# Lumina-Group/libzkp

Hardware: AMD Instinct MI355X
Metric: proofs/sec (whole node) + ms/proof p50, 4096-proof mixed batch (range / equality / membership / improvement) per MI355X (higher is better)
Workload: dtype u32/u64 integer limbs (10x25.5-bit GF(2^255-19), BN254 Fq on 9x29-bit limbs in the MSM loops and 10x26-bit elsewhere, 8x32-bit Fr and scalars mod l, 2x64-bit f128)

## Files before the change

### libzkp_amd/csrc/g16_impl.inc

```

namespace {

struct G16Key {
    bool loaded = false;
    uint32_t n_inst = 0, n_wit = 0, nv = 0, n_rows = 0, m = 0, logm = 0;
    G16Circuit C{};
    std::vector<void*> allocs;
    uint32_t *table_g1 = nullptr, *table_g2 = nullptr;
    G16Radix rx = g16_radix(G16_WBITS_DEFAULT);
    int shared_tables = -1;
    uint64_t table_bytes = 0;
    struct Chunking { DevLayout lay; const uint32_t* corr = nullptr; const uint16_t* scal = nullptr; };
    std::vector<SlotList> targets_g1, targets_g2;
    std::vector<uint16_t> hscal_g1, hscal_g2;
    std::map<uint64_t, Chunking> lays_g1, lays_g2;
    uint64_t win_g1 = 0, win_g2 = 0;
    const uint32_t *init_g1 = nullptr, *init_g2 = nullptr;
    G16Vk vk{}; bool vk_ready = false;
    uint64_t vk_table_bytes = 0;
    bool verifier_only() const { return vk_ready && !loaded; }
    const uint32_t *vm_kconst = nullptr, *vm_lines = nullptr;
};
struct G16Run {
    void* buf = nullptr; size_t cap = 0; hipStream_t side = nullptr, side2 = nullptr; hipEvent_t ev[4] = {nullptr, nullptr, nullptr, nullptr};
// ... 316 lines not shown
    const HostR1CS cs = kind == G16_EQUALITY ? build_equality_r1cs() : build_membership_r1cs();
    const HostCircuitTables T = build_circuit_tables(cs);
    uint32_t seed[8];
    if (setup_seed) memcpy(seed, setup_seed, 32);
    else { std::vector<uint8_t> f; int rc0 = fresh_seeds(f, 1); if (rc0) return rc0; memcpy(seed, f.data(), 32); }
    const char* tagname = kind == G16_EQUALITY ? "equality_mimc" : "membership_mimc";
    uint8_t th[32]; sha256_host(th, (const uint8_t*)tagname, strlen(tagname));
    const uint32_t tag = (uint32_t)th[0] | ((uint32_t)th[1] << 8) | ((uint32_t)th[2] << 16);
    fr tw[5];
    for (uint32_t k = 0; k < 5; k++) { tw[k] = tape_fr(seed, 0x47313601u, 8 * tag + k); if (fp_is_zero(tw[k])) tw[k] = fp_one<FrParams>(); }
    const fr alpha = tw[0], beta = tw[1], gamma = tw[2], delta = tw[3], tau = tw[4];
    const uint32_t m = T.m, nv = T.nv;
    const fr one = fp_one<FrParams>();
    fr taum = one; for (uint32_t i = 0; i < m; i++) taum = fp_mul(taum, tau);
    const fr zt = fp_sub(taum, one), minv = fp_inv(fp_from_u64<FrParams>(m));
    const fr w = fr9_to_fr<FrParams>(ld_fr9_c(T.tw.data(), 1));
    std::vector<fr> lag(m);
    fr wj = one;
    for (uint32_t j = 0; j < m; j++) { lag[j] = fp_mul(fp_mul(fp_mul(zt, minv), wj), fp_inv(fp_sub(tau, wj))); wj = fp_mul(wj, w); }
    std::vector<fr> At(nv, fp_zero<FrParams>()), Bt = At, Ct = At;
    std::vector<fr>* dst[3] = {&At, &Bt, &Ct};
    for (int q = 0; q < 3; q++)
        for (uint32_t j = 0; j < T.n_rows; j++)
            for (uint32_t e = T.ptr[q][j]; e < T.ptr[q][j + 1]; e++)
                (*dst[q])[T.col[q][e]] = fp_add((*dst[q])[T.col[q][e]], fp_mul(ld_fr_c(T.coef[q].data(), e), lag[j]));
    for (uint32_t i = 0; i < T.n_inst; i++) At[i] = fp_add(At[i], lag[T.n_rows + i]);
    const fr ginv = fp_inv(gamma), dinv = fp_inv(delta);
    auto mix = [&](uint32_t k) { return fp_add(fp_add(fp_mul(beta, At[k]), fp_mul(alpha, Bt[k])), Ct[k]); };
    std::vector<fr> s1 = {alpha, beta, delta}, s2 = {beta, gamma, delta};
    for (uint32_t i = 0; i < T.n_inst; i++) s1.push_back(fp_mul(mix(i), ginv));
    for (uint32_t k = 0; k < nv; k++) s1.push_back(At[k]);
    for (uint32_t k = 0; k < nv; k++) s1.push_back(Bt[k]);
    { fr tp = fp_mul(zt, dinv); for (uint32_t i = 0; i + 1 < m; i++) { s1.push_back(tp); tp = fp_mul(tp, tau); } }
    for (uint32_t k = T.n_inst; k < nv; k++) s1.push_back(fp_mul(mix(k), dinv));
    for (uint32_t k = 0; k < nv; k++) s2.push_back(Bt[k]);
    std::vector<uint8_t> b1, b2; int rc;
    if ((rc = gpu_scalar_mults(false, s1, b1)) || (rc = gpu_scalar_mults(true, s2, b2))) return rc;
    auto g1at = [&](size_t i) { return b1.data() + 64 * i; };
    auto g2at = [&](size_t i) { return b2.data() + 128 * i; };
    auto put = [](std::vector<uint8_t>& v, const uint8_t* p, size_t n) { v.insert(v.end(), p, p + n); };
    auto put_len = [](std::vector<uint8_t>& v, uint64_t n) { for (int i = 0; i < 8; i++) v.push_back((uint8_t)(n >> (8 * i))); };
    size_t o_abc = 3, o_a = o_abc + T.n_inst, o_b = o_a + nv, o_h = o_b + nv, o_l = o_h + (m - 1);
    vk.clear();
    put(vk, g1at(0), 64); put(vk, g2at(0), 128); put(vk, g2at(1), 128); put(vk, g2at(2), 128);
    put_len(vk, T.n_inst); put(vk, g1at(o_abc), 64ull * T.n_inst);
    pk = vk;
    put(pk, g1at(1), 64); put(pk, g1at(2), 64);
    put_len(pk, nv); put(pk, g1at(o_a), 64ull * nv);
    put_len(pk, nv); put(pk, g1at(o_b), 64ull * nv);
    put_len(pk, nv); put(pk, g2at(3), 128ull * nv);
    put_len(pk, m - 1); put(pk, g1at(o_h), 64ull * (m - 1));
    put_len(pk, T.n_wit); put(pk, g1at(o_l), 64ull * T.n_wit);
    return load_key_locked(kind, pk.data(), pk.size());
}

int launch_msm_key(bool g2, const G16Radix& rx, const G16Key::Chunking& ch, const uint32_t* table, const uint32_t* acc_init, uint32_t rows, const uint32_t* digits, uint32_t* partial, hipStream_t st) {
    const DevLayout& D = ch.lay;
    const MsmView m = g16_msm_view(rx, D, ch.scal, table, acc_init, rows, digits, partial);
    Device::KProf& K = dev().prof[g2 ? 2 : 1];
    hipEvent_t e1 = nullptr;
    int rc = prof_begin(K, st, &e1);
    if (rc) return rc;
    ZKP_TRACED(g2 ? "k_msm_gather<G2Msm>" : "k_msm_gather<G1Msm>", st, g16_launch_msm(g2, m, st));
    prof_end(K, st, e1, D.adds_per_row * rows);
    return 0;
}


int run_g16(int kind, uint32_t rows, const uint64_t* d_value, const uint64_t* d_set_vals, const uint32_t* d_set_len, const uint8_t* d_seeds,
            uint8_t* d_out, uint64_t stride, hipStream_t st, uint32_t lane = 0) {
    G16Key& K = g16s().key[kind];
    if (!K.loaded) return no_proving_key(K);
    const uint32_t nsc = g16_nscalars(K.nv, K.m);
    const G16Key::Chunking *c1 = nullptr, *c1c = nullptr, *c2 = nullptr;
    int rc;
    if ((rc = get_chunking(K, false, G16_PART_AB, rows, &c1)) || (rc = get_chunking(K, true, G16_PART_ALL, rows, &c2))) return rc;
    if ((rc = get_chunking(K, false, G16_PART_C, rows, &c1c))) return rc;
    size_t off = 0;
    auto sz = [&](size_t bytes) { size_t o = off; off += align_up(bytes); return o; };
    const size_t W = (size_t)32 * rows;
    const size_t o_z = sz(W * K.nv), o_sd = sz((size_t)K.rx.digw * 4 * rows * nsc), o_rs = sz(W * 2), o_p1 = sz((size_t)c1->lay.nchunks * G1_JAC_W * 4 * rows),
                 o_p1c = sz((size_t)c1c->lay.nchunks * G1_JAC_W * 4 * rows), o_p2 = sz((size_t)c2->lay.nchunks * G2_JAC_W * 4 * rows),
                 o_s1 = sz((size_t)3 * G1_JAC_W * 4 * rows), o_s2 = sz((size_t)G2_JAC_W * 4 * rows), o_t1 = sz((size_t)G16_CPARTS * G1_JAC_W * 4 * rows),
                 o_qe = sz((size_t)2 * 9 * K.m * 4 * rows);
    G16Run& RW = g16s().run[kind][lane & 1u];
    if (off > RW.cap) {
        if (RW.buf) { HIP_TRY(hipDeviceSynchronize()); HIP_TRY(hipFree(RW.buf)); RW.buf = nullptr; RW.cap = 0; }
        HIP_TRY(hipMalloc(&RW.buf, off)); RW.cap = off;
    }
    uint8_t* base = (uint8_t*)RW.buf;
    G16View V{}; V.rx = K.rx; V.rows = rows; V.kind = (uint32_t)kind; V.n_inst = K.n_inst; V.n_wit = K.n_wit; V.nv = K.nv; V.m = K.m;
    V.value = d_value; V.set_vals = d_set_vals; V.set_len = d_set_len; V.seeds = reinterpret_cast<const uint32_t*>(d_seeds); V.mimc_c = g16s().mimc_dev;
    V.z = (uint32_t*)(base + o_z); V.sdig = (uint32_t*)(base + o_sd); V.rs = (uint32_t*)(base + o_rs); V.out = d_out; V.stride = stride;
    V.qap_evals = (uint32_t*)(base + o_qe);
    uint32_t *p1 = (uint32_t*)(base + o_p1), *p1c = (uint32_t*)(base + o_p1c), *p2 = (uint32_t*)(base + o_p2), *s1 = (uint32_t*)(base + o_s1), *s2 = (uint32_t*)(base + o_s2), *t1 = (uint32_t*)(base + o_t1);
    if (!RW.last) {
        for (auto& e : RW.ev) HIP_TRY(hipEventCreateWithFlags(&e, hipEventDisableTiming));
        HIP_TRY(hipEventCreateWithFlags(&RW.last, hipEventDisableTiming));
    }
    G16Run& R0 = g16s().run[kind][0];
    if (!R0.side) {
        static const int side_level = env_int("ZKP_HIP_G16_SIDE_PRIORITY", 2), side2_level = env_int("ZKP_HIP_G16_SIDE2_PRIORITY", 0);
        HIP_TRY(hipStreamCreateWithPriority(&R0.side, hipStreamNonBlocking, stream_priority(side_level)));
        HIP_TRY(hipStreamCreateWithPriority(&R0.side2, hipStreamNonBlocking, stream_priority(side2_level)));
    }
    hipStream_t const side = R0.side, side2 = R0.side2;
    hipEvent_t ev_wit = RW.ev[0], ev_ab = RW.ev[1], ev_c = RW.ev[2], ev_cp = RW.ev[3];
    ReduceView R2{}; R2.rows = rows; R2.ntargets = 1; R2.partial = p2; R2.target_chunk_begin = c2->lay.target_chunk_begin; R2.corr = c2->corr;
    if (RW.used) HIP_TRY(hipStreamWaitEvent(st, RW.last, 0));
    ZKP_TRACED("k_g16_witness", st, g16_launch_witness(V, st));
    ZKP_TRACED("k_g16_zdigits", st, g16_launch_zdigits(V, st));
    HIP_TRY(hipEventRecord(ev_wit, st));
    HIP_TRY(hipStreamWaitEvent(side, ev_wit, 0));
    { TraceMark tm_("k_g16_qap", side); HIP_TRY(g16_launch_qap(V, K.C, side)); }
    if ((rc = launch_msm_key(false, K.rx, *c1c, K.table_g1, K.init_g1, rows, V.sdig, p1c, side))) return rc;
    ReduceView Rc{}; Rc.rows = rows; Rc.ntargets = 1; Rc.partial = p1c; Rc.target_chunk_begin = c1c->lay.target_chunk_begin; Rc.corr = c1c->corr;
    ZKP_TRACED("k_sum_t<G1Msm>", side, g16_launch_sum(false, Rc, s1 + (size_t)2 * G1_JAC_W * rows, side));
    HIP_TRY(hipEventRecord(ev_c, side));
    if ((rc = launch_msm_key(false, K.rx, *c1, K.table_g1, K.init_g1, rows, V.sdig, p1, st))) return rc;
    ReduceView Rab{}; Rab.rows = rows; Rab.ntargets = 2; Rab.partial = p1; Rab.target_chunk_begin = c1->lay.target_chunk_begin; Rab.corr = c1->corr;
    if (c1->lay.ntargets == 3) Rab.target_chunk_end = c1->lay.target_chunk_begin + 2;
    HIP_TRY(hipEventRecord(ev_ab, st));
    HIP_TRY(hipStreamWaitEvent(side2, ev_ab, 0));
    ZKP_TRACED("k_sum_t<G1Msm>", side2, g16_launch_sum(false, Rab, s1, side2));
    ZKP_TRACED("k_g16_cparts", side2, g16_launch_cparts(V, s1, t1, side2));
    HIP_TRY(hipEventRecord(ev_cp, side2));
    if ((rc = launch_msm_key(true, K.rx, *c2, K.table_g2, K.init_g2, rows, V.sdig, p2, st))) return rc;
    ZKP_TRACED("k_sum_t<G2Msm>", st, g16_launch_sum(true, R2, s2, st));
    HIP_TRY(hipStreamWaitEvent(st, ev_c, 0));
    HIP_TRY(hipStreamWaitEvent(st, ev_cp, 0));
    ZKP_TRACED("k_g16_final", st, g16_launch_final(V, s1, s2, t1, st));
    HIP_TRY(hipGetLastError());
    HIP_TRY(hipEventRecord(RW.last, st)); RW.used = true;
    return 0;
}

int prove_g16_host(int kind, uint64_t n, const uint64_t* values, const uint64_t* sets_flat, const uint32_t* set_counts, const std::vector<uint8_t>& valid,
                   const uint8_t* seeds, uint8_t* out, uint64_t stride, uint32_t* out_len, int32_t* status) {
    if (g16s().key[kind].verifier_only()) return no_proving_key(g16s().key[kind]);
    std::vector<uint64_t> v, sv; std::vector<uint32_t> sl, idx; std::vector<uint8_t> sd;
    size_t pos = 0; int any = 0;
    memset(out, 0, stride * n);
    for (uint64_t i = 0; i < n; i++) {
        const uint32_t cnt = set_counts ? set_counts[i] : 0;
        if (valid[i]) {
            idx.push_back((uint32_t)i); v.push_back(values[i]);
            sd.insert(sd.end(), seeds + 32 * i, seeds + 32 * i + 32);
            if (kind == G16_MEMBERSHIP) { sl.push_back(cnt); for (uint32_t k = 0; k < G16_MAX_SET; k++) sv.push_back(k < cnt ? sets_flat[pos + k] : 0); }
            const uint32_t plen = kind == G16_EQUALITY ? EQUALITY_ENVELOPE_BYTES : (uint32_t)membership_envelope_bytes(cnt);
            if (plen > stride) return fail(ZKP_HIP_E_ARGUMENT, "stride too small for the proof envelope");
            out_len[i] = plen; status[i] = ZKP_HIP_OK;
        } else { out_len[i] = 0; status[i] = ZKP_HIP_INVALID_INPUT; any = 1; }
        pos += cnt;
    }
    const uint32_t rows = (uint32_t)idx.size();
    if (rows == 0) return any;
    hipStream_t st = dev().stream;
    uint64_t *d_v = nullptr, *d_sv = nullptr; uint32_t* d_sl = nullptr; uint8_t *d_sd = nullptr, *d_out = nullptr;
    DevScope mem;
    HIP_TRY(mem.alloc(&d_v, 8ull * rows)); HIP_TRY(mem.alloc(&d_sd, 32ull * rows)); HIP_TRY(mem.alloc(&d_out, stride * rows));
    HIP_TRY(hipMemcpyAsync(d_v, v.data(), 8ull * rows, hipMemcpyHostToDevice, st));
    HIP_TRY(hipMemcpyAsync(d_sd, sd.data(), 32ull * rows, hipMemcpyHostToDevice, st));
    HIP_TRY(hipMemsetAsync(d_out, 0, stride * rows, st));
    if (kind == G16_MEMBERSHIP) {
        HIP_TRY(mem.alloc(&d_sv, 8ull * sv.size())); HIP_TRY(mem.alloc(&d_sl, 4ull * rows));
        HIP_TRY(hipMemcpyAsync(d_sv, sv.data(), 8ull * sv.size(), hipMemcpyHostToDevice, st));
        HIP_TRY(hipMemcpyAsync(d_sl, sl.data(), 4ull * rows, hipMemcpyHostToDevice, st));
// ... 284 lines not shown
```

### libzkp_amd/csrc/g16_kernels.hip

```cpp
#include "g16_launch.h"
#include "msm_kernel.h"

struct G1Msm {
    static constexpr uint32_t ACC_W = G1_JAC_W, DIG_PER_WORD = 2;
    static __device__ __forceinline__ int32_t digit(uint32_t word, uint32_t w) { return (int32_t)(int16_t)(word >> (16 * (w & 1u))); }
    using Acc = g1_jac;
    static __device__ __forceinline__ Acc identity() { return jac_infinity<fq>(); }
    static constexpr uint32_t GATHER_WAVES = 3; static constexpr int GATHER_PREFETCH = 2;
    static constexpr uint32_t GATHER_W = 16, GATHER_STRIDE = 16, GATHER_PRIO = 0;
    using GAcc = g1_xyzz9;
    static __device__ __forceinline__ GAcc to_gather(const g1_jac& a) { return xyzz9_from_jac(a); }
    static __device__ __forceinline__ g1_jac from_gather(const GAcc& a) { return jac_from_xyzz9(a); }
    static __device__ __forceinline__ GAcc accumulate_entry(const GAcc& acc, int32_t d, const uint32_t* e) {
        g1_aff9 q{fq9_unpack8(e), fq9_unpack8(e + 8)};
        q.y = fq9_select(d < 0, fq9_neg_k<4>(q.y), q.y);
        return g1_mmadd9(acc, q);
    }
    static __device__ __forceinline__ void store(uint32_t* p, uint32_t idx, uint32_t row, uint32_t rows, const Acc& a) { st_g1_jac(p, idx, row, rows, a); }
    static __device__ __forceinline__ Acc load(const uint32_t* p, uint32_t idx, uint32_t row, uint32_t rows) { return ld_g1_jac(p, idx, row, rows); }
    static __device__ __forceinline__ Acc add(const Acc& a, const Acc& b) { return jac_add(a, b); }
};
struct G2Msm {
    static constexpr uint32_t ACC_W = G2_JAC_W, DIG_PER_WORD = 2;
    static __device__ __forceinline__ int32_t digit(uint32_t word, uint32_t w) { return (int32_t)(int16_t)(word >> (16 * (w & 1u))); }
    using Acc = g2_jac;
    static __device__ __forceinline__ Acc identity() { return jac_infinity<fq2>(); }
    static constexpr uint32_t GATHER_WAVES = 2; static constexpr int GATHER_PREFETCH = -1;
    static constexpr uint32_t GATHER_W = 32, GATHER_STRIDE = 32, GATHER_PRIO = 0;
    using GAcc = g2_xyzz9;
    static __device__ __forceinline__ GAcc to_gather(const g2_jac& a) { return g2_xyzz9_from_jac(a); }
    static __device__ __forceinline__ g2_jac from_gather(const GAcc& a) { return jac_from_g2_xyzz9(a); }
    static __device__ __forceinline__ GAcc accumulate_entry(const GAcc& acc, int32_t d, const uint32_t* e) {
        const g2_aff9 q{fq2_9{fq9_unpack8(e), fq9_unpack8(e + 8)}, fq2_9{fq9_unpack8(e + 16), fq9_unpack8(e + 24)}};
        return g2_mmadd9(acc, q, d < 0);
    }
    static __device__ __forceinline__ void store(uint32_t* p, uint32_t idx, uint32_t row, uint32_t rows, const Acc& a) { st_g2_jac(p, idx, row, rows, a); }
    static __device__ __forceinline__ Acc load(const uint32_t* p, uint32_t idx, uint32_t row, uint32_t rows) { return ld_g2_jac(p, idx, row, rows); }
    static __device__ __forceinline__ Acc add(const Acc& a, const Acc& b) { return jac_add(a, b); }
};


__global__ void __launch_bounds__(TW) k_g16_witness(G16View V) {
    ZKP_RAISE_PRIO();
    const uint32_t row = blockIdx.x * TW + threadIdx.x;
    if (row < V.rows) step_g16_witness(V, row);
}
__global__ void __launch_bounds__(TB) k_g16_zdigits(G16View V) {
    ZKP_RAISE_PRIO();
    const uint32_t row = blockIdx.x * TB + threadIdx.x;
    if (row < V.rows) step_g16_zdigits(V, blockIdx.y, row);
}
struct DevSync { __device__ __forceinline__ void operator()() const { __syncthreads(); } };
static constexpr int QAP_TB_MAX = 256;
__global__ void __launch_bounds__(QAP_TB_MAX) k_g16_qap(G16View V, G16Circuit C) {
    extern __shared__ uint32_t g16_lds[];
    G16Lds L; L.base = g16_lds; L.m = C.m;
    g16_qap_proof(V, C, L, V.qap_evals + (size_t)blockIdx.x * 2 * 9 * C.m, blockIdx.x, threadIdx.x, blockDim.x, DevSync());
}
__global__ void __launch_bounds__(TW) k_g16_cparts(G16View V, const uint32_t* sum_g1, uint32_t* tmp_g1) {
    ZKP_RAISE_PRIO();
    const uint32_t row = blockIdx.x * TW + threadIdx.x;
    if (row < V.rows) step_g16_cparts(V, sum_g1, tmp_g1, blockIdx.y, row);
}
__global__ void __launch_bounds__(TW) k_g16_final(G16View V, const uint32_t* sum_g1, const uint32_t* sum_g2, const uint32_t* tmp_g1) {
    ZKP_RAISE_PRIO();
    const uint32_t row = blockIdx.x * TW + threadIdx.x;
    if (row < V.rows) step_g16_final(V, sum_g1, sum_g2, tmp_g1, blockIdx.y, row);
}
__global__ void __launch_bounds__(TW) k_mimc_commit(const uint64_t* values, uint32_t n, const uint32_t* mimc_c, uint8_t* out) {
    const uint32_t i = blockIdx.x * TW + threadIdx.x;
    if (i >= n) return;
    G16View V{}; V.mimc_c = mimc_c; V.z = nullptr;
    const fr h = g16_mimc_chain(V, 0, fp_from_u64<FrParams>(values[i]), 0);
    uint32_t w[8]; fp_to_raw(w, h);
    g16_put_bytes(out + 32ull * i, w, 8);
}
constexpr uint32_t G16_TABLE_SEG = 512;
template <class F, uint32_t AFF_W>
__global__ void __launch_bounds__(TW, 2) k_g16_build_table(const uint32_t* bases, uint32_t nslots, uint32_t* table, uint32_t fmt9, G16Radix rx) {
    const uint32_t seg_len = rx.nent < G16_TABLE_SEG ? rx.nent : G16_TABLE_SEG, nseg = rx.nent / seg_len, slot_seg = rx.slot_ent / seg_len;
    const uint32_t t = blockIdx.x * TW + threadIdx.x;
    if (t >= nslots * slot_seg) return;
    const uint32_t slot = t / slot_seg, sg = t % slot_seg;
    uint32_t win = sg / nseg, seg = sg % nseg;
    if (rx.uneven && sg >= 16u * nseg) { win = sg < 18u * nseg ? 16u : 17u; seg = sg - (win == 16u ? 16u : 18u) * nseg; }
    constexpr uint32_t FW = AFF_W / 2, BATCH = 8;
    Aff<F> base;
    {
        const uint32_t* b = bases + (size_t)slot * AFF_W;
        uint32_t* bx = reinterpret_cast<uint32_t*>(&base.x); uint32_t* by = reinterpret_cast<uint32_t*>(&base.y);
        for (uint32_t k = 0; k < FW; k++) { bx[k] = b[k]; by[k] = b[FW + k]; }
    }
    Jac<F> q = jac_from_aff(base);
    for (uint32_t i = 0; i < g16_win_bit(rx, win); i++) q = jac_dbl(q);
    Jac<F> acc = q;
    {
        const uint32_t first = seg * seg_len + 1;
        int top = 31; while (top > 0 && !((first >> top) & 1u)) top--;
        for (int b = top - 1; b >= 0; b--) { acc = jac_dbl(acc); if ((first >> b) & 1u) acc = jac_add(acc, q); }
    }
    constexpr uint32_t NC = AFF_W / 10;
    const uint32_t OW = fmt9 ? 8 * NC : AFF_W;
    uint32_t* dst = table + ((size_t)slot * rx.slot_ent + g16_win_off(rx, win) + (size_t)seg * seg_len) * OW;
    for (uint32_t e0 = 0; e0 < seg_len; e0 += BATCH) {
        Jac<F> pts[BATCH]; F zp[BATCH];
        for (uint32_t k = 0; k < BATCH; k++) {
            pts[k] = acc; acc = jac_add(acc, q);
            zp[k] = k ? f_mul(zp[k - 1], pts[k].Z) : pts[k].Z;
        }
        F inv = f_inv(zp[BATCH - 1]);
        for (int k = BATCH - 1; k >= 0; k--) {
            const F zi = k ? f_mul(inv, zp[k - 1]) : inv;
            if (k) inv = f_mul(inv, pts[k].Z);
            const F zi2 = f_sq(zi);
            Aff<F> a; a.x = f_mul(pts[k].X, zi2); a.y = f_mul(pts[k].Y, f_mul(zi2, zi));
            const uint32_t* ax = reinterpret_cast<const uint32_t*>(&a.x); const uint32_t* ay = reinterpret_cast<const uint32_t*>(&a.y);
            uint32_t* o = dst + (size_t)(e0 + k) * OW;
            if (fmt9) {
                const fq* c = reinterpret_cast<const fq*>(&a);
                for (uint32_t t2 = 0; t2 < NC; t2++) fq9_pack8(o + 8 * t2, fq9_from_fq(c[t2]));
                continue;
            }
            for (uint32_t j = 0; j < FW; j++) { o[j] = ax[j]; o[FW + j] = ay[j]; }
        }
    }
}



__global__ void __launch_bounds__(TW) k_g16_serialize(bool g2, const uint32_t* jac, uint32_t rows, uint8_t* out) {
    const uint32_t row = blockIdx.x * TW + threadIdx.x;
    if (row >= rows) return;
    if (!g2) { uint32_t w[16]; g1_serialize(w, ld_g1_jac(jac, 0, row, rows)); g16_put_bytes(out + 64ull * row, w, 16); }
    else { uint32_t w[32]; g2_serialize(w, ld_g2_jac(jac, 0, row, rows)); g16_put_bytes(out + 128ull * row, w, 32); }
}

template __global__ void k_msm_gather<G1Msm>(MsmView, uint32_t, uint32_t);
template __global__ void k_msm_gather<G2Msm>(MsmView, uint32_t, uint32_t);
static constexpr uint32_t G16_SUM_ROWS = 8, G16_SUM_TB = 256;
template __global__ void k_sum_t<G1Msm, G16_SUM_ROWS, G16_SUM_TB>(ReduceView, uint32_t*);
template __global__ void k_sum_t<G2Msm, G16_SUM_ROWS, G16_SUM_TB>(ReduceView, uint32_t*);
template __global__ void k_g16_build_table<fq, 20>(const uint32_t*, uint32_t, uint32_t*, uint32_t, G16Radix);
template __global__ void k_g16_build_table<fq2, 40>(const uint32_t*, uint32_t, uint32_t*, uint32_t, G16Radix);

void g16_launch_witness(const G16View& V, hipStream_t st) { k_g16_witness<<<(V.rows + TW - 1) / TW, TW, 0, st>>>(V); }
void g16_launch_zdigits(const G16View& V, hipStream_t st) { k_g16_zdigits<<<dim3((V.rows + TB - 1) / TB, V.nv), TB, 0, st>>>(V); }
hipError_t g16_launch_qap(const G16View& V, const G16Circuit& C, hipStream_t st) {
    const size_t lds = (size_t)9 * C.m * 4;
    const uint32_t tb = C.m / 4;
    if (tb < 64 || tb > (uint32_t)QAP_TB_MAX || (tb & 63u)) return hipErrorInvalidValue;
    k_g16_qap<<<V.rows, tb, lds, st>>>(V, C);
    return hipSuccess;
}
void g16_launch_cparts(const G16View& V, const uint32_t* sum_g1, uint32_t* tmp_g1, hipStream_t st) {
    k_g16_cparts<<<dim3((V.rows + TW - 1) / TW, G16_CPARTS), TW, 0, st>>>(V, sum_g1, tmp_g1);
}
void g16_launch_final(const G16View& V, const uint32_t* sum_g1, const uint32_t* sum_g2, const uint32_t* tmp_g1, hipStream_t st) {
    k_g16_final<<<dim3((V.rows + TW - 1) / TW, 3), TW, 0, st>>>(V, sum_g1, sum_g2, tmp_g1);
}
void g16_launch_mimc(const uint64_t* values, uint32_t n, const uint32_t* mimc_c, uint8_t* out, hipStream_t st) { k_mimc_commit<<<(n + TW - 1) / TW, TW, 0, st>>>(values, n, mimc_c, out); }
void g16_launch_build_table(bool g2, const uint32_t* bases, uint32_t nslots, uint32_t* table, hipStream_t st, bool msm_form, const G16Radix& rx) {
    const uint32_t seg_len = rx.nent < G16_TABLE_SEG ? rx.nent : G16_TABLE_SEG;
    const uint32_t threads = nslots * (rx.slot_ent / seg_len);
    if (!g2) k_g16_build_table<fq, 20><<<(threads + TW - 1) / TW, TW, 0, st>>>(bases, nslots, table, msm_form ? 1u : 0u, rx);
    else k_g16_build_table<fq2, 40><<<(threads + TW - 1) / TW, TW, 0, st>>>(bases, nslots, table, msm_form ? 1u : 0u, rx);
}
uint32_t g16_table_entry_words(bool g2, bool msm_form) { return msm_form ? (g2 ? G2Msm::GATHER_W : G1Msm::GATHER_W) : (g2 ? 40u : 20u); }
uint32_t g16_msm_rows_per_block(bool) { return 256u; }
uint32_t g16_msm_blocks_per_cu(bool g2) { return g2 ? G2Msm::GATHER_WAVES : G1Msm::GATHER_WAVES; }
void g16_launch_msm(bool g2, const MsmView& m, hipStream_t st) {
    const uint32_t ngroups = (m.rows + 255u) / 256u, nblocks = m.nchunks * ngroups, grid = ((nblocks + 7) / 8) * 8;
    if constexpr (gather_lds_bytes<G2Msm>() > 0 || gather_lds_bytes<G1Msm>() > 0) {
        if (gather_lds_bytes<G1Msm>()) (void)hipFuncSetAttribute(reinterpret_cast<const void*>(k_msm_gather<G1Msm>), hipFuncAttributeMaxDynamicSharedMemorySize, (int)gather_lds_bytes<G1Msm>());
        if (gather_lds_bytes<G2Msm>()) (void)hipFuncSetAttribute(reinterpret_cast<const void*>(k_msm_gather<G2Msm>), hipFuncAttributeMaxDynamicSharedMemorySize, (int)gather_lds_bytes<G2Msm>());
    }
    if (!g2) k_msm_gather<G1Msm><<<grid, 256, gather_lds_bytes<G1Msm>(), st>>>(m, ngroups, nblocks);
    else k_msm_gather<G2Msm><<<grid, 256, gather_lds_bytes<G2Msm>(), st>>>(m, ngroups, nblocks);
}
void g16_launch_sum(bool g2, const ReduceView& R, uint32_t* sums, hipStream_t st) {
    const dim3 grid((R.rows + G16_SUM_ROWS - 1) / G16_SUM_ROWS, R.ntargets);
    if (!g2) k_sum_t<G1Msm, G16_SUM_ROWS, G16_SUM_TB><<<grid, G16_SUM_TB, 0, st>>>(R, sums);
    else k_sum_t<G2Msm, G16_SUM_ROWS, G16_SUM_TB><<<grid, G16_SUM_TB, 0, st>>>(R, sums);
}
void g16_launch_serialize(bool g2, const uint32_t* jac, uint32_t rows, uint8_t* out, hipStream_t st) { k_g16_serialize<<<(rows + TW - 1) / TW, TW, 0, st>>>(g2, jac, rows, out); }
```

### libzkp_amd/csrc/g16_steps.h

```cpp
#pragma once
#include "bn254_g.h"
#include "bn254_fr9.h"
#include "keccak.h"
#include "sc25519.h"

namespace zkp {

struct G16Radix { uint32_t wbits, nwin, nent, digw, nwin_u64, uneven, slot_ent; };
constexpr uint32_t G16_UNEVEN_TOP_ENT = 25088;
ZKP_HD inline G16Radix g16_radix(uint32_t wbits, bool uneven = false) {
    G16Radix r; r.wbits = wbits; r.nwin = (254 + wbits) / wbits; r.nent = 1u << (wbits - 1); r.nwin_u64 = (64 + wbits) / wbits; r.uneven = 0;
    r.slot_ent = r.nwin * r.nent;
    if (uneven && wbits == 14) { r.uneven = 1; r.nwin = 18; r.slot_ent = 18u * r.nent + G16_UNEVEN_TOP_ENT; }
    r.digw = (r.nwin + 1) / 2;
    return r;
}
ZKP_HD inline uint32_t g16_win_bit(const G16Radix& rx, uint32_t w) { return rx.uneven && w == 17 ? 239u : rx.wbits * w; }
ZKP_HD inline uint32_t g16_win_off(const G16Radix& rx, uint32_t w) { return (w + (rx.uneven && w == 17 ? 1u : 0u)) * rx.nent; }
ZKP_HD inline uint32_t g16_win_ent(const G16Radix& rx, uint32_t w) { return !rx.uneven || w < 16 ? rx.nent : w == 16 ? 2u * rx.nent : G16_UNEVEN_TOP_ENT; }
constexpr uint32_t G16_WBITS_DEFAULT = 14, G16_WBITS_KNEE = 13, G16_WBITS_MIN = 8, G16_WBITS_MAX = 15, G16_DIGW_MAX = 16;
static_assert(G16_WBITS_DEFAULT >= G16_WBITS_MIN && G16_WBITS_DEFAULT <= G16_WBITS_MAX, "key-table radix out of range");
ZKP_HD inline void g16_recode_uneven(uint32_t* packed, const sc& raw) {
    uint32_t carry = 0;
    ZKP_UNROLL for (int j = 0; j < 18; j++) {
        const int bit = j == 17 ? 239 : 14 * j, wb = j < 16 ? 14 : 15, wd = bit >> 5, sh = bit & 31;
        uint32_t x = wd < 8 ? raw.v[wd] >> sh : 0u;
        if (sh + wb > 32 && wd + 1 < 8) x |= raw.v[wd + 1] << (32 - sh);
        uint32_t d = (x & ((1u << wb) - 1u)) + carry;
        carry = j < 17 && d > (1u << (wb - 1)) ? 1u : 0u;
        d = (d - (carry << wb)) & 0xffffu;
        if ((j & 1) == 0) packed[j >> 1] = d; else packed[j >> 1] |= d << 16;
    }
}
ZKP_HD inline void g16_recode(uint32_t* packed, const sc& raw, const G16Radix& rx) {
    if (rx.uneven) { g16_recode_uneven(packed, raw); return; }
    switch (rx.wbits) {
        case 8: sc_recode_signed<8, 32>(packed, raw); break;
        case 9: sc_recode_signed<9, 29>(packed, raw); break;
        case 10: sc_recode_signed<10, 26>(packed, raw); break;
        case 11: sc_recode_signed<11, 24>(packed, raw); break;
        case 12: sc_recode_signed<12, 22>(packed, raw); break;
        case 13: sc_recode_signed<13, 20>(packed, raw); break;
        case 14: sc_recode_signed<14, 19>(packed, raw); break;
        default: sc_recode_signed<15, 17>(packed, raw); break;
    }
}
constexpr uint32_t G16V_WBITS = 10, G16V_NWIN = 26, G16V_NENT = 512, G16V_NWIN_U64 = 7;

constexpr uint32_t MIMC_ROUNDS = 110, G16_MAX_SET = 64;
constexpr uint32_t G16_TAPE_IDX = 0x47313600u;
enum { G16_EQUALITY = 0, G16_MEMBERSHIP = 1 };

ZKP_HD inline fr ld_fr(const uint32_t* p, uint32_t idx, uint32_t row, uint32_t rows) {
    fr r; const uint32_t* q = p + (size_t)idx * 8 * rows + row;
    ZKP_UNROLL for (int k = 0; k < 8; k++) r.v[k] = q[(size_t)k * rows];
    return r;
}
ZKP_HD inline void st_fr(uint32_t* p, uint32_t idx, uint32_t row, uint32_t rows, const fr& s) {
    uint32_t* q = p + (size_t)idx * 8 * rows + row;
    ZKP_UNROLL for (int k = 0; k < 8; k++) q[(size_t)k * rows] = s.v[k];
}
ZKP_HD inline fr ld_fr_c(const uint32_t* p, uint32_t idx) { fr r; ZKP_UNROLL for (int k = 0; k < 8; k++) r.v[k] = p[(size_t)idx * 8 + k]; return r; }
ZKP_HD inline void g16_put_bytes(uint8_t* dst, const uint32_t* w, int nwords) {
    for (int i = 0; i < nwords; i++) { dst[4 * i] = (uint8_t)w[i]; dst[4 * i + 1] = (uint8_t)(w[i] >> 8); dst[4 * i + 2] = (uint8_t)(w[i] >> 16); dst[4 * i + 3] = (uint8_t)(w[i] >> 24); }
}
ZKP_HD inline void st_fr_digits(uint32_t* d, uint32_t idx, uint32_t row, uint32_t rows, const fr& x, const G16Radix& rx) {
    sc raw; fp_to_raw(raw.v, x);
    uint32_t pk[G16_DIGW_MAX]; g16_recode(pk, raw, rx);
    uint32_t* q = d + (size_t)idx * rx.digw * rows + row;
    ZKP_UNROLL for (uint32_t k = 0; k < G16_DIGW_MAX; k++) if (k < rx.digw) q[(size_t)k * rows] = pk[k];
}

struct G16View {
    uint32_t rows, kind;
    G16Radix rx;
    uint32_t n_inst, n_wit, nv, m;
    const uint64_t* value;
    const uint64_t* set_vals;
    const uint32_t* set_len;
    const uint32_t* seeds;
    const uint32_t* mimc_c;
    uint32_t* z;
    uint32_t* sdig;
    uint32_t* rs;
    uint32_t* qap_evals;
    uint8_t* out; uint64_t stride;
};
ZKP_HD inline uint32_t g16_sc_h(const G16View& V) { return V.nv; }
ZKP_HD inline uint32_t g16_sc_r(const G16View& V) { return V.nv + V.m - 1; }
ZKP_HD inline uint32_t g16_sc_s(const G16View& V) { return V.nv + V.m; }
ZKP_HD inline uint32_t g16_sc_nrs(const G16View& V) { return V.nv + V.m + 1; }
ZKP_HD inline uint32_t g16_sc_one(const G16View& V) { return V.nv + V.m + 2; }
ZKP_HD inline uint32_t g16_nscalars(uint32_t nv, uint32_t m) { return nv + m + 3; }

ZKP_HD inline fr g16_mimc_chain(const G16View& V, uint32_t row, fr x, uint32_t wit0) {
    for (uint32_t i = 0; i < MIMC_ROUNDS; i++) {
        const fr t = fp_add(x, ld_fr_c(V.mimc_c, i));
        const fr t2 = fp_sq(t), t4 = fp_sq(t2);
        x = fp_mul(t4, t);
        if (V.z) { st_fr(V.z, wit0 + 3 * i, row, V.rows, t2); st_fr(V.z, wit0 + 3 * i + 1, row, V.rows, t4); st_fr(V.z, wit0 + 3 * i + 2, row, V.rows, x); }
    }
    return x;
}

ZKP_HD inline void step_g16_witness(const G16View& V, uint32_t row) {
    const uint32_t rows = V.rows;
    const uint64_t val = V.value[row];
    const fr one = fp_one<FrParams>(), zero = fp_zero<FrParams>();
    const fr v = fp_from_u64<FrParams>(val);
    uint8_t* o = V.out + (uint64_t)row * V.stride;
    st_fr(V.z, 0, row, rows, one);
    fr h;
    uint32_t proof_len = 256;
    if (V.kind == G16_EQUALITY) {
        st_fr(V.z, 2, row, rows, v); st_fr(V.z, 3, row, rows, v);
        h = g16_mimc_chain(V, row, v, 4);
        st_fr(V.z, 1, row, rows, h);
        o[0] = 2; o[1] = 2;
    } else {
        const uint32_t len = V.set_len[row];
        const uint64_t* sv = V.set_vals + (size_t)row * G16_MAX_SET;
        const uint32_t w0 = V.n_inst;
        st_fr(V.z, w0, row, rows, v);
        h = g16_mimc_chain(V, row, v, w0 + 1);
        st_fr(V.z, 1, row, rows, h);
        uint32_t pos = 0xffffffffu;
        for (uint32_t i = 0; i < len; i++) if (pos == 0xffffffffu && sv[i] == val) pos = i;
        const uint32_t sel0 = w0 + 1 + 3 * MIMC_ROUNDS;
        for (uint32_t i = 0; i < G16_MAX_SET; i++) {
            const bool real = i < len;
            const fr si = fp_from_u64<FrParams>(real ? sv[i] : 0);
            st_fr(V.z, 2 + i, row, rows, si);
            st_fr(V.z, 2 + G16_MAX_SET + i, row, rows, real ? one : zero);
            const bool sel = i == pos;
            st_fr(V.z, sel0 + i, row, rows, sel ? one : zero);
            st_fr(V.z, sel0 + G16_MAX_SET + i, row, rows, (sel && !real) ? one : zero);
            st_fr(V.z, sel0 + 2 * G16_MAX_SET + i, row, rows, sel ? fp_sub(v, si) : zero);
        }
        o[0] = 2; o[1] = 4;
        proof_len = 4 + 8 * len + 256;
        uint8_t* pl = o + 10;
        pl[0] = (uint8_t)len; pl[1] = (uint8_t)(len >> 8); pl[2] = (uint8_t)(len >> 16); pl[3] = (uint8_t)(len >> 24);
        for (uint32_t i = 0; i < len; i++) for (int k = 0; k < 8; k++) pl[4 + 8 * i + k] = (uint8_t)(sv[i] >> (8 * k));
    }
    for (int k = 0; k < 4; k++) { o[2 + k] = (uint8_t)(proof_len >> (8 * k)); o[6 + k] = (uint8_t)(32u >> (8 * k)); }
    uint32_t hraw[8]; fp_to_raw(hraw, h);
    g16_put_bytes(o + 10 + proof_len, hraw, 8);
    uint32_t seed[8]; ZKP_UNROLL for (int k = 0; k < 8; k++) seed[k] = V.seeds[(size_t)row * 8 + k];
    uint32_t w[16];
    tape_draw64(w, seed, G16_TAPE_IDX, 0); const fr r = fp_from_wide<FrParams>(w);
    tape_draw64(w, seed, G16_TAPE_IDX, 1); const fr s = fp_from_wide<FrParams>(w);
    st_fr_digits(V.sdig, g16_sc_r(V), row, rows, r, V.rx);
    st_fr_digits(V.sdig, g16_sc_s(V), row, rows, s, V.rx);
    st_fr_digits(V.sdig, g16_sc_nrs(V), row, rows, fp_neg(fp_mul(r, s)), V.rx);
    uint32_t* q = V.sdig + (size_t)g16_sc_one(V) * V.rx.digw * rows + row;
// ... 39 lines not shown
        else if (is_one) acc = fp_add(acc, ld_fr(z, c, row, rows));
        else acc = fp_add(acc, fp_mul(cf, ld_fr(z, c, row, rows)));
    }
    return acc;
}
ZKP_HD inline void g16_qap_load(const G16View& V, const G16Circuit& C, const G16Lds& L, uint32_t poly, uint32_t row, uint32_t tid, uint32_t nthreads) {
    const uint32_t nc = C.n_rows;
    const uint32_t *ptr = poly == 0 ? C.a_ptr : poly == 1 ? C.b_ptr : C.c_ptr, *col = poly == 0 ? C.a_col : poly == 1 ? C.b_col : C.c_col,
                   *coef = poly == 0 ? C.a_coef : poly == 1 ? C.b_coef : C.c_coef;
    for (uint32_t j = tid; j < C.m; j += nthreads) {
        fr a = fp_zero<FrParams>();
        if (j < nc) a = g16_row_dot_fast(ptr, col, coef, j, V.z, row, V.rows);
        else if (poly == 0 && j < nc + V.n_inst) a = ld_fr(V.z, j - nc, row, V.rows);
        L.st(j, fr9_from_fr(a));
    }
}
ZKP_HD inline void g16_bf_dif(fr9& u, fr9& v, const fr9& w) { const fr9 s = fr9_reduce_weak(fr9_add(u, v)); v = fr9_mul(fr9_sub_k<4>(u, v), w); u = s; }
ZKP_HD inline void g16_bf_dit(fr9& u, fr9& v, const fr9& w) { const fr9 t = fr9_mul(v, w); v = fr9_sub_k<2>(u, t); u = fr9_add(u, t); }
template <bool DIF>
ZKP_HD inline void g16_stage_single(const G16Circuit& C, const G16Lds& L, const uint32_t* tw, uint32_t half, uint32_t tid, uint32_t nthreads) {
    const uint32_t len = 2 * half, tstride = C.m / len;
    for (uint32_t k = tid; k < C.m / 2; k += nthreads) {
        const uint32_t grp = k / half, j = k % half, i0 = grp * len + j, i1 = i0 + half;
        const fr9 w = ld_fr9_c(tw, j * tstride);
        fr9 u = L.ld(i0), v = L.ld(i1);
        if (DIF) g16_bf_dif(u, v, w); else g16_bf_dit(u, v, w);
        L.st(i0, u); L.st(i1, v);
    }
}
template <bool DIF>
ZKP_HD inline void g16_stage_pair(const G16Circuit& C, const G16Lds& L, const uint32_t* tw, uint32_t h, uint32_t tid, uint32_t nthreads) {
    const uint32_t s1 = C.m / (2 * h), s2 = C.m / (4 * h);
    for (uint32_t q = tid; q < C.m / 4; q += nthreads) {
        const uint32_t grp = q / h, j = q % h, e0 = grp * 4 * h + j;
        fr9 x0 = L.ld(e0), x1 = L.ld(e0 + h), x2 = L.ld(e0 + 2 * h), x3 = L.ld(e0 + 3 * h);
        const fr9 wh = ld_fr9_c(tw, j * s1), wa = ld_fr9_c(tw, j * s2), wb = ld_fr9_c(tw, (j + h) * s2);
        if (DIF) { g16_bf_dif(x0, x2, wa); g16_bf_dif(x1, x3, wb); g16_bf_dif(x0, x1, wh); g16_bf_dif(x2, x3, wh); }
        else { g16_bf_dit(x0, x1, wh); g16_bf_dit(x2, x3, wh); g16_bf_dit(x0, x2, wa); g16_bf_dit(x1, x3, wb); }
        L.st(e0, x0); L.st(e0 + h, x1); L.st(e0 + 2 * h, x2); L.st(e0 + 3 * h, x3);
    }
}
template <class Sync> ZKP_HD inline void g16_transform_dif(const G16Circuit& C, const G16Lds& L, const uint32_t* tw, uint32_t tid, uint32_t nthreads, Sync sync) {
    uint32_t half = C.m / 2;
    if (C.logm & 1u) { g16_stage_single<true>(C, L, tw, half, tid, nthreads); sync(); half >>= 1; }
    for (; half >= 2; half >>= 2) { g16_stage_pair<true>(C, L, tw, half / 2, tid, nthreads); sync(); }
}
template <class Sync> ZKP_HD inline void g16_transform_dit(const G16Circuit& C, const G16Lds& L, const uint32_t* tw, uint32_t tid, uint32_t nthreads, Sync sync) {
    uint32_t h = 1;
    for (uint32_t i = 0; i < C.logm / 2; i++, h <<= 2) { g16_stage_pair<false>(C, L, tw, h, tid, nthreads); sync(); }
    if (C.logm & 1u) { g16_stage_single<false>(C, L, tw, C.m / 2, tid, nthreads); sync(); }
}
ZKP_HD inline void g16_scale_bitrev(const G16Circuit& C, const G16Lds& L, const uint32_t* tab, uint32_t tid, uint32_t nthreads) {
    for (uint32_t p = tid; p < C.m; p += nthreads) L.st(p, fr9_mul(L.ld(p), ld_fr9_c(tab, g16_bitrev(p, C.logm))));
}
ZKP_HD inline void g16_spill(const G16Circuit& C, const G16Lds& L, uint32_t* dst, uint32_t tid, uint32_t nthreads) {
    for (uint32_t w = tid; w < 9 * C.m; w += nthreads) dst[w] = L.base[w];
}
ZKP_HD inline fr9 g16_ld_spilled(const uint32_t* src, uint32_t m, uint32_t e) { fr9 r; const uint32_t p = G16Lds::sw(e); ZKP_UNROLL for (int k = 0; k < 9; k++) r.v[k] = src[(size_t)k * m + p]; return r; }
ZKP_HD inline void g16_pointwise(const G16Circuit& C, const G16Lds& L, const uint32_t* ea, const uint32_t* eb, uint32_t tid, uint32_t nthreads) {
    const fr9 zinv = ld_fr9_c(C.zinv, 0);
    for (uint32_t i = tid; i < C.m; i += nthreads)
        L.st(i, fr9_mul(fr9_sub_k<32>(fr9_mul(g16_ld_spilled(ea, C.m, i), g16_ld_spilled(eb, C.m, i)), L.ld(i)), zinv));
}
ZKP_HD inline void g16_store_h_bitrev(const G16View& V, const G16Circuit& C, const G16Lds& L, uint32_t row, uint32_t tid, uint32_t nthreads) {
    for (uint32_t p = tid; p < C.m; p += nthreads) {
        const uint32_t i = g16_bitrev(p, C.logm);
        if (i + 1 < C.m) st_fr_digits(V.sdig, g16_sc_h(V) + i, row, V.rows, fr9_to_fr<FrParams>(fr9_mul(L.ld(p), ld_fr9_c(C.coset_inv, i))), V.rx);
    }
}
template <class Sync>
ZKP_HD inline void g16_qap_proof(const G16View& V, const G16Circuit& C, const G16Lds& L, uint32_t* scratch, uint32_t row, uint32_t tid, uint32_t nthreads, Sync sync) {
    for (uint32_t poly = 0; poly < 3; poly++) {
        g16_qap_load(V, C, L, poly, row, tid, nthreads); sync();
        g16_transform_dif(C, L, C.tw_inv, tid, nthreads, sync);
        g16_scale_bitrev(C, L, C.coset, tid, nthreads); sync();
        g16_transform_dit(C, L, C.tw, tid, nthreads, sync);
        if (poly < 2) { g16_spill(C, L, scratch + (size_t)poly * 9 * C.m, tid, nthreads); sync(); }
    }
    g16_pointwise(C, L, scratch, scratch + (size_t)9 * C.m, tid, nthreads); sync();
    g16_transform_dif(C, L, C.tw_inv, tid, nthreads, sync);
    g16_store_h_bitrev(V, C, L, row, tid, nthreads);
}

#define G1_JAC_W 30
#define G2_JAC_W 60
ZKP_HD inline fq ld_fq_col(const uint32_t* q, uint32_t rows) { fq r; ZKP_UNROLL for (int k = 0; k < 10; k++) r.v[k] = q[(size_t)k * rows]; return r; }
ZKP_HD inline void st_fq_col(uint32_t* q, uint32_t rows, const fq& a) { ZKP_UNROLL for (int k = 0; k < 10; k++) q[(size_t)k * rows] = a.v[k]; }
ZKP_HD inline g1_jac ld_g1_jac(const uint32_t* p, uint32_t idx, uint32_t row, uint32_t rows) {
    const uint32_t* q = p + (size_t)idx * G1_JAC_W * rows + row; const size_t s = (size_t)10 * rows;
    g1_jac r; r.X = ld_fq_col(q, rows); r.Y = ld_fq_col(q + s, rows); r.Z = ld_fq_col(q + 2 * s, rows);
    return r;
}
ZKP_HD inline void st_g1_jac(uint32_t* p, uint32_t idx, uint32_t row, uint32_t rows, const g1_jac& g) {
    uint32_t* q = p + (size_t)idx * G1_JAC_W * rows + row; const size_t s = (size_t)10 * rows;
    st_fq_col(q, rows, g.X); st_fq_col(q + s, rows, g.Y); st_fq_col(q + 2 * s, rows, g.Z);
}
ZKP_HD inline g2_jac ld_g2_jac(const uint32_t* p, uint32_t idx, uint32_t row, uint32_t rows) {
    const uint32_t* q = p + (size_t)idx * G2_JAC_W * rows + row; const size_t s = (size_t)10 * rows;
    g2_jac r;
    r.X.c0 = ld_fq_col(q, rows); r.X.c1 = ld_fq_col(q + s, rows); r.Y.c0 = ld_fq_col(q + 2 * s, rows); r.Y.c1 = ld_fq_col(q + 3 * s, rows);
    r.Z.c0 = ld_fq_col(q + 4 * s, rows); r.Z.c1 = ld_fq_col(q + 5 * s, rows);
    return r;
}
ZKP_HD inline void st_g2_jac(uint32_t* p, uint32_t idx, uint32_t row, uint32_t rows, const g2_jac& g) {
    uint32_t* q = p + (size_t)idx * G2_JAC_W * rows + row; const size_t s = (size_t)10 * rows;
    st_fq_col(q, rows, g.X.c0); st_fq_col(q + s, rows, g.X.c1); st_fq_col(q + 2 * s, rows, g.Y.c0); st_fq_col(q + 3 * s, rows, g.Y.c1);
    st_fq_col(q + 4 * s, rows, g.Z.c0); st_fq_col(q + 5 * s, rows, g.Z.c1);
}
constexpr uint32_t G16_CPARTS = 4;
ZKP_HD inline void step_g16_cparts(const G16View& V, const uint32_t* sum_g1, uint32_t* tmp_g1, uint32_t part, uint32_t row) {
    const uint32_t rows = V.rows, which = part >> 1;
    g1_jac P = ld_g1_jac(sum_g1, which, row, rows);
    const fr k = ld_fr(V.rs, which == 0 ? 1 : 0, row, rows);
    glv_half h1, h2; fr_glv_split(k.v, h1, h2);
    if (part & 1u) P.X = fq_mul(P.X, fq_glv_beta());
    const glv_half& h = (part & 1u) ? h2 : h1;
    st_g1_jac(tmp_g1, part, row, rows, jac_mul_u128_signed(P, h.mag, h.neg));
}
ZKP_HD inline void step_g16_final(const G16View& V, const uint32_t* sum_g1, const uint32_t* sum_g2, const uint32_t* tmp_g1, uint32_t which, uint32_t row) {
    const uint32_t rows = V.rows;
    uint8_t* o = V.out + (uint64_t)row * V.stride;
    uint32_t plen = 0; for (int k = 0; k < 4; k++) plen |= (uint32_t)o[2 + k] << (8 * k);
    uint8_t* pr = o + 10 + plen - 256;
    if (which == 0) {
        uint32_t w1[16]; g1_serialize(w1, ld_g1_jac(sum_g1, 0, row, rows)); g16_put_bytes(pr, w1, 16);
    } else if (which == 1) {
        uint32_t w2[32]; g2_serialize(w2, ld_g2_jac(sum_g2, 0, row, rows)); g16_put_bytes(pr + 64, w2, 32);
    } else {
        g1_jac Cc = ld_g1_jac(sum_g1, 2, row, rows);
        for (uint32_t t = 0; t < G16_CPARTS; t++) Cc = jac_add(Cc, ld_g1_jac(tmp_g1, t, row, rows));
        uint32_t w1[16]; g1_serialize(w1, Cc); g16_put_bytes(pr + 192, w1, 16);
    }
}

}
```

Before: 341,200.

## Run QAP NTTs in registers per wavefront with shuffle exchanges

Replaces the LDS-based block QAP transform with a single-wavefront kernel that holds each polynomial's evaluations in registers and moves data between lanes with __shfl_xor. A compile-time schedule is used to minimise the number of exchanges. The work is split into three launches (per-polynomial forward and inverse transforms, then pointwise and inverse) so the three polynomials run in parallel across grid.y. Scratch grows to three polys per row, and the new path carries heavy register pressure plus extra global round trips.

```diff
diff --git a/libzkp_amd/csrc/g16_impl.inc b/libzkp_amd/csrc/g16_impl.inc
--- a/libzkp_amd/csrc/g16_impl.inc
+++ b/libzkp_amd/csrc/g16_impl.inc
@@ -422,7 +422,7 @@
     const size_t o_z = sz(W * K.nv), o_sd = sz((size_t)K.rx.digw * 4 * rows * nsc), o_rs = sz(W * 2), o_p1 = sz((size_t)c1->lay.nchunks * G1_JAC_W * 4 * rows),
                  o_p1c = sz((size_t)c1c->lay.nchunks * G1_JAC_W * 4 * rows), o_p2 = sz((size_t)c2->lay.nchunks * G2_JAC_W * 4 * rows),
                  o_s1 = sz((size_t)3 * G1_JAC_W * 4 * rows), o_s2 = sz((size_t)G2_JAC_W * 4 * rows), o_t1 = sz((size_t)G16_CPARTS * G1_JAC_W * 4 * rows),
-                 o_qe = sz((size_t)2 * 9 * K.m * 4 * rows);
+                 o_qe = sz((size_t)G16_QAP_BLOCKS * 9 * K.m * 4 * rows);
     G16Run& RW = g16s().run[kind][lane & 1u];
     if (off > RW.cap) {
         if (RW.buf) { HIP_TRY(hipDeviceSynchronize()); HIP_TRY(hipFree(RW.buf)); RW.buf = nullptr; RW.cap = 0; }
diff --git a/libzkp_amd/csrc/g16_kernels.hip b/libzkp_amd/csrc/g16_kernels.hip
--- a/libzkp_amd/csrc/g16_kernels.hip
+++ b/libzkp_amd/csrc/g16_kernels.hip
@@ -55,7 +55,81 @@
 __global__ void __launch_bounds__(QAP_TB_MAX) k_g16_qap(G16View V, G16Circuit C) {
     extern __shared__ uint32_t g16_lds[];
     G16Lds L; L.base = g16_lds; L.m = C.m;
-    g16_qap_proof(V, C, L, V.qap_evals + (size_t)blockIdx.x * 2 * 9 * C.m, blockIdx.x, threadIdx.x, blockDim.x, DevSync());
+    g16_qap_proof(V, C, L, V.qap_evals + (size_t)blockIdx.x * G16_QAP_BLOCKS * 9 * C.m, blockIdx.x, threadIdx.x, blockDim.x, DevSync());
+}
+template <uint32_t N, uint32_t I = 0, class F> __device__ __forceinline__ void g16_wave_each(F&& f) {
+    if constexpr (I < N) { f(std::integral_constant<uint32_t, I>()); g16_wave_each<N, I + 1>(f); }
+}
+template <uint32_t LOGM, bool DIF, uint32_t S, uint32_t I = 0>
+__device__ __forceinline__ void g16_wave_stage(fr9 (&x)[G16Wave<LOGM>::E], const uint32_t* tw, uint32_t lane, fr9& w) {
+    using W = G16Wave<LOGM>;
+    if constexpr (I < W::E / 2) {
+        constexpr typename W::Stage st = W::stage(DIF, S);
+        if constexpr (st.k >= 0) {
+            const fr9 mine = W::give(st, x, lane, I);
+            fr9 got; ZKP_UNROLL for (int k = 0; k < 9; k++) got.v[k] = __shfl_xor(mine.v[k], 1 << st.k);
+            W::take(st, x, lane, I, got);
+        }
+        constexpr bool fresh = I == 0 || W::tw_index(st, 0, I) != W::tw_index(st, 0, I == 0 ? 0 : I - 1);
+        if constexpr (fresh) w = ld_fr9_c(tw, W::tw_index(st, lane, I));
+        W::template butterfly<DIF>(st, x, I, w);
+        __builtin_amdgcn_sched_barrier(0);
+        g16_wave_stage<LOGM, DIF, S, I + 1>(x, tw, lane, w);
+    }
+}
+template <uint32_t LOGM, bool DIF, uint32_t S = 0>
+__device__ __forceinline__ void g16_wave_transform(fr9 (&x)[G16Wave<LOGM>::E], const uint32_t* tw, uint32_t lane) {
+    if constexpr (S < LOGM) {
+        fr9 w;
+        g16_wave_stage<LOGM, DIF, S>(x, tw, lane, w);
+        g16_wave_transform<LOGM, DIF, S + 1>(x, tw, lane);
+    }
+}
+template <uint32_t LOGM, uint32_t PHASE>
+__global__ void __launch_bounds__(64, LOGM == 10 ? 2 : 3) k_g16_qap_wave(G16View V, G16Circuit C) {
+    using W = G16Wave<LOGM>;
+    constexpr uint32_t E = W::E;
+    constexpr typename W::Map m0 = W::map0(), m1 = W::map1();
+    const uint32_t row = blockIdx.x, lane = threadIdx.x, poly = PHASE == 2 ? 2u : blockIdx.y;
+    uint32_t* scratch = V.qap_evals + (size_t)row * G16_QAP_BLOCKS * 9 * W::M, *mine = scratch + (size_t)poly * 9 * W::M;
+    if constexpr (PHASE == 0) {
+        _Pragma("nounroll") for (uint32_t s = 0; s < E; s++) {
+            const fr9 f = g16_qap_element(V, C, poly, row, W::pos(m0, lane, s));
+            ZKP_UNROLL for (uint32_t k = 0; k < 9; k++) mine[g16_wave_scratch_at(s, k, lane)] = f.v[k];
+        }
+    }
+    fr9 x[E];
+    g16_wave_each<E>([&](auto s) __attribute__((always_inline)) { ZKP_UNROLL for (uint32_t k = 0; k < 9; k++) x[s].v[k] = mine[g16_wave_scratch_at(s, k, lane)]; });
+    if constexpr (PHASE == 0) {
+        g16_wave_transform<LOGM, true>(x, C.tw_inv, lane);
+        g16_wave_each<E>([&](auto s) __attribute__((always_inline)) {
+            x[s] = fr9_mul(x[s], ld_fr9_c(C.coset, g16_bitrev(W::pos(m1, lane, s), LOGM)));
+            __builtin_amdgcn_sched_barrier(0);
+        });
+    } else if constexpr (PHASE == 1) {
+        g16_wave_transform<LOGM, false>(x, C.tw, lane);
+    } else {
+        const fr9 zinv = ld_fr9_c(C.zinv, 0);
+        g16_wave_each<E>([&](auto s) __attribute__((always_inline)) {
+            fr9 a, b;
+            ZKP_UNROLL for (uint32_t k = 0; k < 9; k++) { a.v[k] = scratch[g16_wave_scratch_at(s, k, lane)]; b.v[k] = scratch[9 * W::M + g16_wave_scratch_at(s, k, lane)]; }
+            x[s] = fr9_mul(fr9_sub_k<32>(fr9_mul(a, b), x[s]), zinv);
+            __builtin_amdgcn_sched_barrier(0);
+        });
+        g16_wave_transform<LOGM, true>(x, C.tw_inv, lane);
+    }
+    g16_wave_each<E>([&](auto s) __attribute__((always_inline)) { ZKP_UNROLL for (uint32_t k = 0; k < 9; k++) mine[g16_wave_scratch_at(s, k, lane)] = x[s].v[k]; });
+    if constexpr (PHASE == 2) {
+        _Pragma("nounroll") for (uint32_t s = 0; s < E; s++) {
+            fr9 f; ZKP_UNROLL for (uint32_t k = 0; k < 9; k++) f.v[k] = mine[g16_wave_scratch_at(s, k, lane)];
+            g16_store_h_element(V, C, row, W::pos(m1, lane, s), f);
+        }
+    }
+}
+template <uint32_t LOGM> static void g16_launch_qap_wave(const G16View& V, const G16Circuit& C, hipStream_t st) {
+    k_g16_qap_wave<LOGM, 0><<<dim3(V.rows, 3), 64, 0, st>>>(V, C);
+    k_g16_qap_wave<LOGM, 1><<<dim3(V.rows, 3), 64, 0, st>>>(V, C);
+    k_g16_qap_wave<LOGM, 2><<<dim3(V.rows, 1), 64, 0, st>>>(V, C);
 }
 __global__ void __launch_bounds__(TW) k_g16_cparts(G16View V, const uint32_t* sum_g1, uint32_t* tmp_g1) {
     ZKP_RAISE_PRIO();
@@ -146,6 +220,9 @@
 void g16_launch_witness(const G16View& V, hipStream_t st) { k_g16_witness<<<(V.rows + TW - 1) / TW, TW, 0, st>>>(V); }
 void g16_launch_zdigits(const G16View& V, hipStream_t st) { k_g16_zdigits<<<dim3((V.rows + TB - 1) / TB, V.nv), TB, 0, st>>>(V); }
 hipError_t g16_launch_qap(const G16View& V, const G16Circuit& C, hipStream_t st) {
+    if (C.m != (1u << C.logm)) return hipErrorInvalidValue;
+    if (C.logm == 9) { g16_launch_qap_wave<9>(V, C, st); return hipSuccess; }
+    if (C.logm == 10) { g16_launch_qap_wave<10>(V, C, st); return hipSuccess; }
     const size_t lds = (size_t)9 * C.m * 4;
     const uint32_t tb = C.m / 4;
     if (tb < 64 || tb > (uint32_t)QAP_TB_MAX || (tb & 63u)) return hipErrorInvalidValue;
diff --git a/libzkp_amd/csrc/g16_steps.h b/libzkp_amd/csrc/g16_steps.h
--- a/libzkp_amd/csrc/g16_steps.h
+++ b/libzkp_amd/csrc/g16_steps.h
@@ -71,6 +71,7 @@
     ZKP_UNROLL for (uint32_t k = 0; k < G16_DIGW_MAX; k++) if (k < rx.digw) q[(size_t)k * rows] = pk[k];
 }
 
+constexpr uint32_t G16_QAP_BLOCKS = 3;
 struct G16View {
     uint32_t rows, kind;
     G16Radix rx;
@@ -276,6 +277,82 @@
     g16_store_h_bitrev(V, C, L, row, tid, nthreads);
 }
 
+template <uint32_t LOGM> struct G16Wave {
+    static_assert(LOGM >= 7 && LOGM <= 10, "6 lane bits and 1 .. 4 slot bits");
+    static constexpr uint32_t LOGE = LOGM - 6, E = 1u << LOGE, M = 1u << LOGM, LANE = 8;
+    struct Map { uint32_t loc[LOGM]; };
+    struct Stage { uint32_t pbit; int32_t k; uint32_t t; Map map; };
+    static constexpr Map map0() { Map m{}; for (uint32_t b = 0; b < LOGM; b++) m.loc[b] = b < 6 ? LANE + b : b - 6; return m; }
+    static constexpr Stage run(Map m, bool dif, uint32_t want) {
+        uint32_t fifo[LOGE] = {}, n = 0;
+        for (uint32_t s = 0; s < LOGM; s++) {
+            Stage st{dif ? LOGM - 1 - s : s, -1, 0, m};
+            const uint32_t b = st.pbit;
+            if (m.loc[b] < LANE) {
+                st.t = m.loc[b];
+                uint32_t j = 0; for (uint32_t i = 0; i < n; i++) if (fifo[i] != st.t) fifo[j++] = fifo[i];
+                fifo[j] = st.t; n = j + 1;
+            } else {
+                st.k = (int32_t)(m.loc[b] - LANE); st.t = n ? fifo[0] : 0;
+                for (uint32_t q = 0; q < LOGM; q++) if (m.loc[q] == st.t) m.loc[q] = LANE + (uint32_t)st.k;
+                m.loc[b] = st.t;
+                for (uint32_t i = 0; i + 1 < n; i++) fifo[i] = fifo[i + 1];
+                if (n) fifo[n - 1] = st.t; else fifo[n++] = st.t;
+            }
+            st.map = m;
+            if (s == want) return st;
+        }
+        return Stage{0, -1, 0, m};
+    }
+    static constexpr Map map1() { return run(map0(), true, LOGM).map; }
+    static constexpr Stage stage(bool dif, uint32_t s) { return run(dif ? map0() : map1(), dif, s); }
+    static constexpr bool closes() {
+        const Map a = map0(), b = run(map1(), false, LOGM).map;
+        uint32_t nx = 0;
+        for (uint32_t s = 0; s < LOGM; s++) nx += (stage(true, s).k >= 0 ? 1u : 0u) + (stage(false, s).k >= 0 ? 1u : 0u);
+        for (uint32_t q = 0; q < LOGM; q++) if (a.loc[q] != b.loc[q]) return false;
+        return nx == 12;
+    }
+    ZKP_HD static constexpr uint32_t pos(const Map& m, uint32_t lane, uint32_t slot) {
+        uint32_t p = 0;
+        ZKP_UNROLL for (uint32_t b = 0; b < LOGM; b++) p |= ((m.loc[b] < LANE ? slot >> m.loc[b] : lane >> (m.loc[b] - LANE)) & 1u) << b;
+        return p;
+    }
+    ZKP_HD static constexpr uint32_t lo(const Stage& st, uint32_t i) { return ((i >> st.t) << (st.t + 1)) | (i & ((1u << st.t) - 1u)); }
+    ZKP_HD static constexpr uint32_t tw_index(const Stage& st, uint32_t lane, uint32_t i) {
+        return (pos(st.map, lane, lo(st, i)) & ((1u << st.pbit) - 1u)) << (LOGM - 1 - st.pbit);
+    }
+    ZKP_HD static uint32_t pick(bool c, uint32_t a, uint32_t b) { return c ? a : b; }
+    ZKP_HD static fr9 give(const Stage& st, const fr9 (&x)[E], uint32_t lane, uint32_t i) {
+        const bool c = (lane >> st.k) & 1u; const uint32_t l = lo(st, i), h = l | (1u << st.t);
+        fr9 r; ZKP_UNROLL for (int k = 0; k < 9; k++) r.v[k] = pick(c, x[l].v[k], x[h].v[k]);
+        return r;
+    }
+    ZKP_HD static void take(const Stage& st, fr9 (&x)[E], uint32_t lane, uint32_t i, const fr9& got) {
+        const bool c = (lane >> st.k) & 1u; const uint32_t l = lo(st, i), h = l | (1u << st.t);
+        ZKP_UNROLL for (int k = 0; k < 9; k++) { x[l].v[k] = pick(c, got.v[k], x[l].v[k]); x[h].v[k] = pick(c, x[h].v[k], got.v[k]); }
+    }
+    template <bool DIF> ZKP_HD static void butterfly(const Stage& st, fr9 (&x)[E], uint32_t i, const fr9& w) {
+        const uint32_t l = lo(st, i), h = l | (1u << st.t);
+        if (DIF) g16_bf_dif(x[l], x[h], w); else g16_bf_dit(x[l], x[h], w);
+    }
+};
+static_assert(G16Wave<9>::closes() && G16Wave<10>::closes(), "the schedule does not return to its first map in six exchanges per transform");
+ZKP_HD inline fr9 g16_qap_element(const G16View& V, const G16Circuit& C, uint32_t poly, uint32_t row, uint32_t j) {
+    const uint32_t nc = C.n_rows;
+    const uint32_t *ptr = poly == 0 ? C.a_ptr : poly == 1 ? C.b_ptr : C.c_ptr, *col = poly == 0 ? C.a_col : poly == 1 ? C.b_col : C.c_col,
+                   *coef = poly == 0 ? C.a_coef : poly == 1 ? C.b_coef : C.c_coef;
+    fr a = fp_zero<FrParams>();
+    if (j < nc) a = g16_row_dot_fast(ptr, col, coef, j, V.z, row, V.rows);
+    else if (poly == 0 && j < nc + V.n_inst) a = ld_fr(V.z, j - nc, row, V.rows);
+    return fr9_from_fr(a);
+}
+ZKP_HD inline void g16_store_h_element(const G16View& V, const G16Circuit& C, uint32_t row, uint32_t p, const fr9& x) {
+    const uint32_t i = g16_bitrev(p, C.logm);
+    if (i + 1 < C.m) st_fr_digits(V.sdig, g16_sc_h(V) + i, row, V.rows, fr9_to_fr<FrParams>(fr9_mul(x, ld_fr9_c(C.coset_inv, i))), V.rx);
+}
+ZKP_HD inline uint32_t g16_wave_scratch_at(uint32_t s, uint32_t k, uint32_t lane) { return (s * 9u + k) * 64u + lane; }
+
 #define G1_JAC_W 30
 #define G2_JAC_W 60
 ZKP_HD inline fq ld_fq_col(const uint32_t* q, uint32_t rows) { fq r; ZKP_UNROLL for (int k = 0; k < 10; k++) r.v[k] = q[(size_t)k * rows]; return r; }
```

After: 338,500. About the same (-0.8%).
